# samuel-watson/glmmrMCML

Hardware: AMD Instinct MI355X
Metric: MCML iters/sec x m chains (simlik evals/sec) (higher is better)
Workload: dtype f64

## Files before the change

glmmrmcml_amd/csrc/ctx.h:

```cpp
#pragma once
#include "common.h"
#include "chol.h"
#include "covspec.h"
#include "band_plan.h"
#include "component_plan.h"
#include "step_ahead.h"

namespace mcml {

typedef int (*reduce_fn)(void* user, double* dev_buf, int n);

enum { KERNEL_SKINNY = 0, KERNEL_BAND = 1, KERNEL_DLDS = 2, KERNEL_REG = 3, KERNEL_SPARSE = 4, KERNEL_COMPONENT = 5,
       KERNEL_EXACT = 6,
       KERNEL_EXACT_COMPONENT = 7 };

struct StepRing {
    static constexpr int SLOTS = StepAhead::SLOTS;
    unsigned long long* h = nullptr;
    unsigned long long* d = nullptr;
    unsigned seq = 0;
    StepRing() = default;
    StepRing(const StepRing&) = delete;
    StepRing& operator=(const StepRing&) = delete;
    ~StepRing() { if (h) (void)hipHostFree(h); }
};

struct HmcState {
    StepRing ring;
    int C = 0;
    int Cw = 0;
    DevMat V, R, UP, GRAD, GRADP;
    DevMat MU, S;
    DevBuf chain;
    DevBuf partial;
    int partial_slots = 0;
    bool cm = false;
    DevBuf cm_part, cm_acc;
    DevBuf cm_part_fwd;
    DevMat LX, ZS;
    DevBuf cp_part;
};

constexpr int NUTS_MAXD = 12;
struct NutsState {
    DevMat vecs[16 + 4 * (NUTS_MAXD + 1)];
    DevBuf chain, part;
};

struct SparseZL {
    bool possible = false, active = false, built = false;
    int W = 0;
    long nnz = 0;
    DevBuf ell_col, ell_src, ell_z, ell_val;
    DevBuf csr_ptr, csr_i, csr_pos, csr_val;
    DevBuf row_start;
    bool factored = false;
    long nnz_z = 0, nnz_l = 0;
    DevBuf zcsr_ptr, zcsr_i, zcsr_val;
    DevBuf row_end;
    DevBuf blk_ptr;
    int nblk = 0, max_blk = 0;
};

struct ComponentDev {
    ComponentPlan plan;
    bool ready = false;
    DevBuf item_ptr, var_ptr, vars, slot_ptr, slot_quarter, slot_i, slot_src, slot_d;
};

struct CompFactors {
    DevBuf fac, fac_ptr, logdet;
    long long doubles = 0;
};

struct KernelProf {
    bool on = false;
    bool skip = false;
    long long seen[4] = {0, 0, 0, 0};
    std::vector<hipEvent_t> ev;
    std::vector<int> kind, e0, e1;
    size_t used = 0, nev = 0;
    int last_stop = -1;
    double ms[4] = {0, 0, 0, 0};
    long long cnt[4] = {0, 0, 0, 0};
    int fresh() {
        if (nev >= ev.size())
            for (int i = 0; i < 512; ++i) { hipEvent_t e; if (hipEventCreate(&e) != hipSuccess) return -1; ev.push_back(e); }
        return (int)nev++;
    }
    int begin(hipStream_t s, int k, bool chain = false) {
        if (!on) return -1;
        ++seen[k];
        if (skip) return -1;
        int st = (chain && last_stop >= 0) ? last_stop : fresh();
        if (st < 0) return -1;
        if (!(chain && last_stop >= 0)) (void)hipEventRecord(ev[st], s);
        if (used >= kind.size()) { kind.resize(used + 512); e0.resize(used + 512); e1.resize(used + 512); }
        kind[used] = k; e0[used] = st; e1[used] = -1;
        return (int)used++;
    }
    void end(hipStream_t s, int slot) {
        if (slot < 0) return;
        const int sp = fresh();
        if (sp < 0) return;
        (void)hipEventRecord(ev[sp], s);
        e1[slot] = sp; last_stop = sp;
    }
    void unchain() { last_stop = -1; }
    void collect() {
        for (size_t i = 0; i < used; ++i) {
            float t = 0;
            if (e1[i] >= 0 && hipEventElapsedTime(&t, ev[e0[i]], ev[e1[i]]) == hipSuccess) { ms[kind[i]] += t; cnt[kind[i]] += 1; }
        }
        used = 0; nev = 0; last_stop = -1;
    }
    ~KernelProf() { for (auto e : ev) (void)hipEventDestroy(e); }
// ... 168 lines not shown
```

glmmrmcml_amd/csrc/hmc.hip:

```cpp
#include <algorithm>
#include <atomic>
#include <chrono>
#include "entry.h"
#include "dgemm_mfma.h"
#include "dgemm_dlds.h"
#include "dgemm_band.h"
#include "dgemm_skinny.h"
#include "glm.h"
#include "reduce.h"
#include "rng.h"
#include "hmc_chain.h"
#include "hmc_cm.h"
#include "hmc_traj.h"

namespace mcml {

template <int FL>
struct EpiForwardT {
    double* MU; double* S; int ld; const double* xb; const double* y; int flink; int store_mu; double var_par;
    __device__ __forceinline__ double score(double yv, double mu) const {
        if constexpr (FL == 12) return glm_score_beta(yv, mu, var_par);
        else return glm_score(yv, mu, FL ? FL : flink);
    }
    __device__ __forceinline__ void elem(int m, int n, double accv) const {
// ... 77 lines not shown
                cb[r] = (size_t)nn * ld;
            }
            double xv[TM][4], rv[TM][4];
#pragma unroll
            for (int i = 0; i < TM; ++i) {
                const int m = mB + 16 * i + (lane & 15);
                const int mm = m < M ? m : 0;
#pragma unroll
                for (int r = 0; r < 4; ++r) {
                    xv[i][r] = Xs[mm + cb[r]];
                    rv[i][r] = mode == 1 ? R[mm + cb[r]] : 0.0;
                }
            }
#pragma unroll
            for (int r = 0; r < 4; ++r) {
                const double en = env[r];
                const bool more = s + 1 < stv[r];
#pragma unroll
                for (int i = 0; i < TM; ++i) {
                    const double x = xv[i][r];
                    double g = -1.0 * x;
                    g = g + post * acc[i][j][r];
                    acc[i][j][r] = g;
                    double rr = rv[i][r];
                    rr = rr + (en / 2) * g;
                    const double rr2 = rr + (en / 2) * g;
                    rr = more ? rr2 : rr;
                    rv[i][r] = rr;
                    xv[i][r] = x + en * rr;
                }
            }
#pragma unroll
            for (int r = 0; r < 4; ++r) {
                const bool act = inN[r] && (mode != 1 || s < stv[r]);
                if (!act) continue;
                const bool more = s + 1 < stv[r];
#pragma unroll
                for (int i = 0; i < TM; ++i) {
                    const int m = mB + 16 * i + (lane & 15);
                    if (m >= M) continue;
                    const size_t off = m + cb[r];
                    if (mode != 1 || !more) G[off] = acc[i][j][r];
                    if (mode == 1) {
                        if (more) UP[off] = xv[i][r];
                        R[off] = rv[i][r];
                    }
                }
            }
        }
    }
};

template <> struct BandFeed<EpiBackward> { static constexpr bool ok = true; };
template <> struct BandFeed<EpiForwardT<1>> { static constexpr bool ok = true; };
template <> struct BandFeed<EpiForwardT<3>> { static constexpr bool ok = true; };
template <> struct BandFeed<EpiForwardT<7>> { static constexpr bool ok = true; };


__global__ __launch_bounds__(256) void k_blockdiag_LV(int Q, int ncols, const int* start, const double* L, int ldl,
                                                      const double* V, int ldv, double* U, int ldu)
{
    const int q = blockIdx.x * 256 + threadIdx.x;
    if (q >= Q) return;
    const int s0 = start[q];
    for (int c = blockIdx.y; c < ncols; c += gridDim.y) {
        const double* v = V + (size_t)c * ldv;
        double acc = 0.0;
        for (int t = s0; t <= q; ++t) acc += L[q + (size_t)t * ldl] * v[t];
        U[q + (size_t)c * ldu] = acc;
    }
}

__global__ __launch_bounds__(256) void k_hmc_init(double* V, int ld, int Q, ChainArrays ca, uint64_t seed,
                                                  uint32_t chain_offset, uint32_t iter_idx, const double* inj_init)
{
    const int c = blockIdx.x;
    const uint32_t gid = chain_offset + (uint32_t)c;
    for (int q = threadIdx.x; q < Q; q += 256)
        V[q + (size_t)c * ld] = inj_init ? inj_init[q + (size_t)c * Q]
                                         : rng_normal(seed, (uint32_t)q, gid, 0u, 16u * iter_idx + 0u);
    if (threadIdx.x == 0) chain_reset(ca, c, seed, gid, iter_idx);
}

template <int FL>
__device__ __forceinline__ double chain_log_prob(const double* MU, int ldm, int n, const double* X, int ldx,
                                                 int Q, const double* y, double var_par, int flink_rt, int c,
                                                 double* sh)
{
    const int flink = FL ? FL : flink_rt;
    double ll = 0, lp = 0;
    for (int i0 = threadIdx.x; i0 < n; i0 += 1024) {
        double m4[4], y4[4];
#pragma unroll
        for (int u = 0; u < 4; ++u) {
            const int i = i0 + 256 * u;
            m4[u] = i < n ? MU[i + (size_t)c * ldm] : 0.0;
            y4[u] = i < n ? y[i] : 0.0;
        }
#pragma unroll
        for (int u = 0; u < 4; ++u)
            if (i0 + 256 * u < n) ll += glm_logpdf(y4[u], m4[u], var_par, flink);
    }
    for (int k0 = threadIdx.x; k0 < Q; k0 += 1024) {
        double x4[4];
#pragma unroll
        for (int u = 0; u < 4; ++u) { const int k = k0 + 256 * u; x4[u] = k < Q ? X[k + (size_t)c * ldx] : 0.0; }
#pragma unroll
        for (int u = 0; u < 4; ++u)
            if (k0 + 256 * u < Q) lp += glm_logpdf(x4[u], 0, 1, 7);
    }
    double a = block_sum(ll, sh);
    double b = block_sum(lp, sh);
    return a + b;
}

template <int FL>
__global__ __launch_bounds__(256) void k_hmc_lp0(const double* MU, int ldm, int n, const double* V, int ld, int Q,
                                                 const double* y, double var_par, int flink, double* lpcur)
{
    __shared__ double sh[4];
    double v = chain_log_prob<FL>(MU, ldm, n, V, ld, Q, y, var_par, flink, blockIdx.x, sh);
    if (threadIdx.x == 0) lpcur[blockIdx.x] = v;
}

__global__ __launch_bounds__(256) void k_hmc_propose(const double* V, const double* GRAD, double* R, double* UP,
                                                     int ld, int Q, ChainArrays ca, double lambda, int max_steps,
                                                     uint64_t seed, uint32_t chain_offset, uint32_t iter_idx,
                                                     int it, const double* inj_mom, int C)
{
    __shared__ double sh[4];
    const int c = blockIdx.x;
    const uint32_t gid = chain_offset + (uint32_t)c;
    const double e = ca.e[c];
    double ss = 0;
    for (int q = threadIdx.x; q < Q; q += 256) {
        const size_t off = q + (size_t)c * ld;
        double r = inj_mom ? inj_mom[q + ((size_t)it * C + c) * Q]
                           : rng_normal(seed, (uint32_t)q, gid, (uint32_t)it, 16u * iter_idx + 2u);
        ss += r * r;
        const double g = GRAD[off], v = V[off];
        r = r + (e / 2) * g;
        R[off] = r;
        UP[off] = v + e * r;
    }
    double tot = block_sum(ss, sh);
    if (threadIdx.x == 0) chain_begin_proposal(ca, c, tot, lambda, max_steps);
}

__global__ void k_max_steps(const int* steps, int C, int* out, unsigned long long* slot = nullptr, unsigned seq = 0)
{
    __shared__ int sh[256];
    int v = 0;
    for (int i = threadIdx.x; i < C; i += 256) v = max(v, steps[i]);
    sh[threadIdx.x] = v;
    __syncthreads();
    for (int o = 128; o > 0; o >>= 1) { if ((int)threadIdx.x < o) sh[threadIdx.x] = max(sh[threadIdx.x], sh[threadIdx.x + o]); __syncthreads(); }
    if (threadIdx.x == 0) {
        out[0] = sh[0];
        if (slot) __hip_atomic_store(slot, ((unsigned long long)seq << 32) | (unsigned)sh[0], __ATOMIC_RELEASE, __HIP_MEMORY_SCOPE_SYSTEM);
    }
}

template <int FL>
__global__ __launch_bounds__(256) void k_hmc_accept(double* V, double* GRAD, const double* R, const double* UP,
                                                    const double* GRADP, int ld, int Q, const double* MU, int ldm,
                                                    int n, const double* y, double var_par, int flink,
                                                    ChainArrays ca, double target_accept, int adapt, int it,
                                                    int C, uint8_t* flags, double* probs)
{
    __shared__ double sh[4];
    __shared__ int acc_s;
    const int c = blockIdx.x;
    double l2 = chain_log_prob<FL>(MU, ldm, n, UP, ld, Q, y, var_par, flink, c, sh);
    double kin = 0;
    for (int k0 = threadIdx.x; k0 < Q; k0 += 1024) {
        double r4[4];
#pragma unroll
        for (int u = 0; u < 4; ++u) { const int k = k0 + 256 * u; r4[u] = k < Q ? R[k + (size_t)c * ld] : 0.0; }
#pragma unroll
        for (int u = 0; u < 4; ++u)
            if (k0 + 256 * u < Q) kin += r4[u] * r4[u];
    }
    kin = block_sum(kin, sh);
    if (threadIdx.x == 0) acc_s = chain_decide(ca, c, l2, kin, target_accept, adapt, it, C, flags, probs);
    __syncthreads();
    const int acc = acc_s;
    if (acc)
        for (int k0 = threadIdx.x; k0 < Q; k0 += 1024) {
            double u4[4], g4[4];
#pragma unroll
            for (int u = 0; u < 4; ++u) {
                const int k = k0 + 256 * u;
                const size_t off = (k < Q ? k : 0) + (size_t)c * ld;
                u4[u] = UP[off]; g4[u] = GRADP[off];
            }
#pragma unroll
            for (int u = 0; u < 4; ++u) {
                const int k = k0 + 256 * u;
                if (k < Q) { const size_t off = k + (size_t)c * ld; V[off] = u4[u]; GRAD[off] = g4[u]; }
            }
        }
}

__global__ __launch_bounds__(256) void k_hmc_store(const double* V, int ld, int Q, double* SAMP, int lds,
                                                   int stride, int col)
{
    const int c = blockIdx.x;
    for (int k = threadIdx.x; k < Q; k += 256) SAMP[k + (size_t)(c * stride + col) * lds] = V[k + (size_t)c * ld];
}

__global__ void k_hmc_diag(ChainArrays ca, int C, double* out)
{
    if (threadIdx.x != 0 || blockIdx.x != 0) return;
    double sa = 0, se = 0, mn = 1e300, mx = 0, ms = 0, sl = 0;
    for (int c = 0; c < C; ++c) {
        sa += ca.acc[c]; se += ca.e[c];
        mn = fmin(mn, ca.e[c]); mx = fmax(mx, ca.e[c]);
        ms = fmax(ms, (double)ca.steps[c]); sl += (double)ca.leap[c];
    }
    out[0] = sa; out[1] = se; out[2] = mn; out[3] = mx; out[4] = ms; out[5] = sl;
}

static bool cm_traj_used(const Ctx& c) { return c.traj_mode == 1 && c.sp.active && c.cp.ready && c.cp.plan.feasible; }

static std::atomic<long long> g_traj_launches{0};
long long cm_traj_launch_count() { return g_traj_launches.load(); }

static int cm_traj_launch(Ctx& c, const TrajArgs& a)
{
    const CompView m = comp_view(c);
    const int waves = cp_waves(c.cp.plan, cp_forced_waves(CP_TRAJ_WAVES_ENV));
    const int lds = cp_lds_bytes(m.max_vars, waves);
    const dim3 grid(m.nitems, cm_chain_blocks(a.C));
    MCML_TRY((dispatch_flink<1, 3, 7, 12>(c.flink, [&](auto FL) {
        if (waves == 4) {
            MCML_TRY(ensure_dynamic_lds((const void*)k_cm_traj<FL(), 4>, cp_lds_bytes(CP_MAX_VARS, 4)));
            hipLaunchKernelGGL((k_cm_traj<FL(), 4>), grid, dim3(256), lds, c.stream, m, a);
        } else {
            MCML_TRY(ensure_dynamic_lds((const void*)k_cm_traj<FL(), 1>, cp_lds_bytes(CP_MAX_VARS, 1)));
            hipLaunchKernelGGL((k_cm_traj<FL(), 1>), grid, dim3(64), lds, c.stream, m, a);
        }
        return (int)MCML_OK;
    })));
    MCML_HIP(hipGetLastError());
    ++g_traj_launches;
    return MCML_OK;
}

static int hmc_alloc(Ctx& c, int C)
{
    HmcState& h = c.hmc;
    h.C = C; h.Cw = C;
    h.cm = c.sp.active;
    auto mat = [&](DevMat& m, int len) { return h.cm ? m.alloc(C, len) : m.alloc(len, C); };
    for (DevMat* m : {&h.V, &h.R, &h.UP, &h.GRAD, &h.GRADP}) MCML_TRY(mat(*m, c.Q));
    MCML_TRY(mat(h.MU, c.n)); MCML_TRY(mat(h.S, c.n));
    MCML_TRY(h.chain.ensure(sizeof(double) * (size_t)round_up(C, 16) * 8));
    if (h.cm) {
        const size_t nchn = (size_t)(c.n + CM_ROWS - 1) / CM_ROWS, nchq = (size_t)(c.Q + cm_qrows(c.Q) - 1) / cm_qrows(c.Q);
        MCML_TRY(h.cm_part.ensure(sizeof(double) * (nchn + 3 * nchq + 4) * (size_t)h.V.ld));
        MCML_TRY(h.cm_acc.ensure(sizeof(int) * (size_t)round_up(C, 64)));
        if (c.sp.factored) { MCML_TRY(h.LX.alloc(C, c.Q)); MCML_TRY(h.ZS.alloc(C, c.Q)); }
        if (cm_traj_used(c)) MCML_TRY(h.cp_part.ensure(sizeof(double) * 4 * (size_t)c.cp.plan.nitems() * h.V.ld));
        return MCML_OK;
    }
    MCML_HIP(hipMemsetAsync(h.V.d(), 0, sizeof(double) * (size_t)h.V.ld * C, c.stream));
    MCML_HIP(hipMemsetAsync(h.UP.d(), 0, sizeof(double) * (size_t)h.UP.ld * C, c.stream));
    MCML_HIP(hipMemsetAsync(h.S.d(), 0, sizeof(double) * (size_t)h.S.ld * C, c.stream));
    return MCML_OK;
}

static bool use_dlds()
{
    static int v = -1;
    if (v < 0) { const char* e = getenv("GLMMR_MCML_GEMM"); v = (e && !strcmp(e, "reg")) ? 0 : 1; }
    return v == 1;
}

static bool use_skinny()
{
    const char* e = getenv("GLMMR_MCML_SKINNY");
    return !(e && !strcmp(e, "0"));
}

struct DenseOp { BandPlan& plan; bool band; int M, K; const DevMat& A; };
template <class Epi>
static int dense_product(Ctx& c, int dir, const DenseOp& a, const double* B, int ldb, const Epi& epi)
{
    const int N = c.hmc.Cw, lda = a.A.ld;
    const double* A = a.A.d();
    if (use_skinny() && skinny_applicable(a.plan, a.M, a.K, N, lda)) {
        c.last_kernel[dir] = KERNEL_SKINNY;
        return launch_skinny(c.stream, a.plan, N, A, lda, B, ldb, epi);
    }
    if (a.band && dlds_applicable(a.M, N, a.K, A, lda, a.A.cols_alloc, B, ldb)) {
        c.last_kernel[dir] = KERNEL_BAND;
        return launch_gemm_band(c.stream, a.plan, N, A, lda, B, ldb, epi);
    }
    if (use_dlds() && dlds_applicable(a.M, N, a.K, A, lda, a.A.cols_alloc, B, ldb)) {
        c.last_kernel[dir] = KERNEL_DLDS;
        return launch_gemm_dlds(c.stream, a.M, N, a.K, A, lda, B, ldb, epi);
    }
    c.last_kernel[dir] = KERNEL_REG;
    return launch_gemm<false>(c.stream, a.M, N, a.K, A, lda, B, ldb, epi);
}

enum : unsigned {
    PROD_STORE_MU = 1,
    PROD_CHAIN = 2,
    PROD_WANT_LL = 4,
    PROD_LX_READY = 8,
};

static int hmc_forward(Ctx& c, const double* X, int ldx, double var_par, unsigned flags = PROD_STORE_MU)
{
    HmcState& h = c.hmc;
    const int store_mu = (flags & PROD_STORE_MU) ? 1 : 0;
    const int slot = c.prof.begin(c.stream, 0, (flags & PROD_CHAIN) != 0);
    int rc;
    if (h.cm) {
        c.last_kernel[0] = KERNEL_SPARSE;
        const int rpw = CM_FR;
        dim3 grid((c.n + 4 * rpw - 1) / (4 * rpw), (h.Cw + 63) / 64);
        int W = c.sp.W; const int* col = c.sp.ell_col.as<int>(); const double* val = c.sp.ell_val.d(); const double* Xin = X;
        if (c.sp.factored) {
            if (!(flags & PROD_LX_READY))
            hipLaunchKernelGGL(k_cm_Lrow, dim3((c.Q + 3) / 4, (h.Cw + 63) / 64), dim3(256), 0, c.stream, c.Q, h.Cw, h.V.ld,
                               c.sp.row_start.as<int>(), c.L.d(), c.L.ld, X, h.LX.d());
            W = c.z_width; col = c.z_idx.as<int>(); val = c.z_val.d(); Xin = h.LX.d();
        }
        double* pll = nullptr;
        if (flags & PROD_WANT_LL) {
            MCML_TRY(h.cm_part_fwd.ensure(sizeof(double) * (size_t)grid.x * h.V.ld));
            pll = h.cm_part_fwd.d();
        }
        dispatch_flink<1, 3, 7, 12>(c.flink, [&](auto FL) {
            hipLaunchKernelGGL((k_cm_forward<FL()>), grid, dim3(256), 0, c.stream, c.n, h.Cw, h.V.ld, W, col, val, Xin, c.xb.d(),
                               c.y.d(), c.flink, var_par, store_mu, h.MU.d(), h.S.d(), rpw, pll, h.V.ld);
        });
        rc = (hipGetLastError() == hipSuccess) ? MCML_OK : MCML_EHIP;
    } else
        rc = dispatch_flink<1, 3, 7, 12>(c.flink, [&](auto FL) {
            return dense_product(c, 0, DenseOp{c.plan_fwd, c.band_fwd, c.n, c.Q, c.ZL}, X, ldx,
                                 EpiForwardT<FL()>{h.MU.d(), h.S.d(), h.MU.ld, c.xb.d(), c.y.d(), c.flink, store_mu, var_par});
        });
    c.prof.end(c.stream, slot);
    return rc;
}

static int hmc_backward(Ctx& c, const double* Xs, double* G, int s, double var_par, int mode, unsigned flags = 0,
                        int next_lx = 0)
{
    HmcState& h = c.hmc;
    ChainArrays ca = chain_arrays(h);
    EpiBackward epi{Xs, G, h.R.d(), h.UP.d(), h.V.ld, ca.e, ca.steps, s, glm_score_post(var_par, c.flink), mode};
    const int slot = c.prof.begin(c.stream, 1, (flags & PROD_CHAIN) != 0);
    int rc;
    if (h.cm) {
        const bool f = c.sp.factored;
        const int* ptr = f ? c.sp.zcsr_ptr.as<int>() : c.sp.csr_ptr.as<int>();
        const int* ci = f ? c.sp.zcsr_i.as<int>() : c.sp.csr_i.as<int>();
        const double* cv = f ? c.sp.zcsr_val.d() : c.sp.csr_val.d();
        double* out = f ? h.ZS.d() : G;
        const int m1 = f ? 2 : mode;
// ... 104 lines not shown
    const int Q = c.Q;
    MCML_TRY(c.U.alloc(Q, ncols));
    MCML_HIP(hipMemsetAsync(c.U.d(), 0, sizeof(double) * (size_t)c.U.ld * ncols, c.stream));
    if (c.sp.active && c.sp.row_start.p) {
        int gy = ncols < 1024 ? ncols : 1024;
        hipLaunchKernelGGL(k_blockdiag_LV, dim3((Q + 255) / 256, gy), dim3(256), 0, c.stream, Q, ncols,
                           c.sp.row_start.as<int>(), c.L.d(), c.L.ld, samp.d(), samp.ld, c.U.d(), c.U.ld);
        MCML_HIP(hipGetLastError());
    } else {
        EpiAxpby epi{c.U.d(), c.U.ld, 1.0, 0.0};
        MCML_TRY(launch_gemm<false>(c.stream, Q, ncols, Q, c.L.d(), c.L.ld, samp.d(), samp.ld, epi));
    }
    c.mcols = ncols;
    c.zu_valid = false; c.uall_valid = false;
    return MCML_OK;
}

}

#include "hmc_exact.h"
#include "hmc_exact_comp.h"

namespace mcml {

bool hmc_exact_applicable(const Ctx& c) { return exact_applicable(c); }
int hmc_exact_sample(Ctx& c, const double* beta, double var_par, const glmmr_mcml_hmc_opts* o, uint64_t seed, uint32_t iter_idx,
                     const double* inj_z, glmmr_mcml_hmc_diag* diag, int* ncols_out)
{
    return exact_gaussian_sample(c, beta, var_par, o, seed, iter_idx, inj_z, nullptr, nullptr, diag, ncols_out);
}

bool hmc_exact_component_applicable(const Ctx& c) { return exact_component_applicable(c); }
int hmc_exact_component_sample(Ctx& c, const double* beta, double var_par, const glmmr_mcml_hmc_opts* o, uint64_t seed,
                               uint32_t iter_idx, const double* inj_z, glmmr_mcml_hmc_diag* diag, int* ncols_out)
{
    return exact_component_sample(c, beta, var_par, o, seed, iter_idx, inj_z, nullptr, nullptr, diag, ncols_out);
}
void hmc_exact_component_sizes(const Ctx& c, long long* out3)
{
    const ComponentPlan& p = c.cp.plan;
    const int waves = cp_waves(p, cp_forced_waves(CP_LA_WAVES_ENV));
    out3[0] = waves; out3[1] = exc_lds_bytes(p.max_vars); out3[2] = 8LL * comp_factor_doubles(c);
}

struct HmcTiming {
    using Clock = std::chrono::steady_clock;
    enum { PROPOSE, LOOK_AHEAD, TRAJECTORY, ACCEPT, NSEG };
    const bool on = enabled();
    Clock::time_point t_phase = Clock::now(), t_mark = t_phase, t_prop = t_phase;
    double setup = 0, loop = 0, sync = 0, slowest = 0, seg[NSEG] = {};
    int n_sync = 0, nprop = 0;

    static bool enabled() { static const bool v = getenv("GLMMR_MCML_HMC_TIMING") != nullptr; return v; }
    static double since(Clock::time_point t) { return std::chrono::duration<double, std::milli>(Clock::now() - t).count(); }
    static double now_ms() { return std::chrono::duration<double, std::milli>(Clock::now().time_since_epoch()).count(); }
    double phase_end() { const double d = since(t_phase); t_phase = Clock::now(); return d; }
    void proposal()
    {
        if (!on) return;
        if (nprop++ > 0) slowest = std::max(slowest, since(t_prop));
        t_prop = t_mark = Clock::now();
    }
    void start() { if (on) t_mark = Clock::now(); }
    void mark(int k) { if (on) { seg[k] = std::max(seg[k], since(t_mark)); t_mark = Clock::now(); } }
    void waited() { if (on) { sync += since(t_mark); ++n_sync; } }
    void print(int total) const
    {
        if (on)
            fprintf(stderr, "hmc_sample: set-up %.2f ms | %d proposals %.2f ms enqueue (%d synchronous, %.2f ms waiting; slowest proposal %.2f ms: propose %.2f, count look-ahead %.2f, trajectory %.2f, accept %.2f) | tail %.2f ms\n",
                    setup, total, loop, n_sync, sync, slowest, seg[PROPOSE], seg[LOOK_AHEAD], seg[TRAJECTORY], seg[ACCEPT], since(t_phase));
    }
};

struct HmcCall {
    const glmmr_mcml_hmc_opts* o; double var_par; uint64_t seed; uint32_t iter_idx;
    SampleShape sh;
    ChainArrays ca;
    const double* mom; uint8_t* flags; double* probs;
    const DevMat* samp;
    int lf;
    double* tpart; size_t tstride;
    StepRing* ring; int* d_maxs;
    bool pending_commit;
    int adapt(int it) const { return (it < o->warmup) && (it < o->adapt); }
};

static void commit_cm(Ctx& c, HmcCall& k, int it)
{
    HmcState& h = c.hmc;
    int stride;
    const bool stores_now = k.sh.column_of(it, &stride) >= 0;
    if (it + 1 < k.sh.total && !stores_now) k.pending_commit = true;
    else hipLaunchKernelGGL(k_cm_commit, dim3((k.sh.C + 63) / 64, cm_parts(c).nchq), dim3(256), 0, c.stream, h.V.d(), h.GRAD.d(),
                            h.UP.d(), h.GRADP.d(), h.V.ld, c.Q, k.sh.C, h.cm_acc.as<int>());
}

static void store_draw(Ctx& c, const HmcCall& k, int it)
{
    int stride;
    const int col = k.sh.column_of(it, &stride);
    if (col >= 0) store_columns(c, *k.samp, stride, col);
}

static int leapfrog_steps(Ctx& c, const HmcCall& k, StepAhead& ahead, HmcTiming& t, int it)
{
    HmcState& h = c.hmc;
    StepRing& ring = *k.ring;
    const unsigned seq = ++ring.seq;
    const int slot = (int)(seq % StepRing::SLOTS);
    hipLaunchKernelGGL(k_max_steps, dim3(1), dim3(256), 0, c.stream, k.ca.steps, k.sh.C, k.d_maxs, ring.d + slot, seq);
    MCML_HIP(hipGetLastError());
    t.mark(HmcTiming::PROPOSE);
    int maxs = ahead.launched(seq, HmcTiming::now_ms);
    if (maxs != StepAhead::SYNCHRONISE) t.mark(HmcTiming::LOOK_AHEAD);
    else {
        t.start();
        MCML_HIP(hipStreamSynchronize(c.stream));
        t.waited();
        maxs = ahead.synchronised(seq);
        MCML_REQUIRE(maxs != StepAhead::NOT_ARRIVED, "hmc: the step count of proposal %d did not arrive (token %llx, expected sequence %u)", it, ring.h[slot], seq);
        MCML_REQUIRE(maxs != StepAhead::OUT_OF_ORDER, "hmc: step-count ring out of order");
    }
    MCML_REQUIRE(maxs >= 1 && maxs <= k.o->max_steps, "hmc: step count %d out of range", maxs);
    c.prof.skip = (it & 3) != 0;
    t.start();
    int rc = MCML_OK;
    for (int s = 0; s < maxs && rc == MCML_OK; ++s) {
        const bool last = s == maxs - 1;
        rc = hmc_forward(c, h.UP.d(), h.UP.ld, k.var_par, (s > 0 ? PROD_CHAIN : 0) | (last ? (h.cm ? PROD_WANT_LL : PROD_STORE_MU) : 0) |
                                                              (k.lf && s > 0 ? PROD_LX_READY : 0));
        if (rc == MCML_OK) rc = hmc_backward(c, h.UP.d(), h.GRADP.d(), s, k.var_par, 1, PROD_CHAIN, last ? 0 : k.lf);
    }
    c.prof.skip = false;
    t.mark(HmcTiming::TRAJECTORY);
    MCML_TRY(rc);
    c.prof.unchain();
    return MCML_OK;
}

static int propose_dense(Ctx& c, HmcCall& k, StepAhead& ahead, HmcTiming& t, int it)
{
    HmcState& h = c.hmc;
    const glmmr_mcml_hmc_opts* o = k.o;
    hipLaunchKernelGGL(k_hmc_propose, dim3(k.sh.C), dim3(256), 0, c.stream, h.V.d(), h.GRAD.d(), h.R.d(), h.UP.d(),
                       h.V.ld, c.Q, k.ca, o->lambda, o->max_steps, k.seed, (uint32_t)o->chain_offset, k.iter_idx, it,
                       k.mom, k.sh.C);
    MCML_TRY(leapfrog_steps(c, k, ahead, t, it));
    dispatch_flink<1, 3, 7>(c.flink, [&](auto FL) {
        hipLaunchKernelGGL((k_hmc_accept<FL()>), dim3(k.sh.C), dim3(256), 0, c.stream, h.V.d(), h.GRAD.d(), h.R.d(), h.UP.d(),
                           h.GRADP.d(), h.V.ld, c.Q, h.MU.d(), h.MU.ld, c.n, c.y.d(), k.var_par, c.flink, k.ca,
                           o->target_accept, k.adapt(it), it, k.sh.C, k.flags, k.probs);
    });
    store_draw(c, k, it);
    MCML_HIP(hipGetLastError());
    t.mark(HmcTiming::ACCEPT);
    return MCML_OK;
}

static int propose_cm(Ctx& c, HmcCall& k, StepAhead& ahead, HmcTiming& t, int it)
{
    HmcState& h = c.hmc;
    const glmmr_mcml_hmc_opts* o = k.o;
    const CmParts p = cm_parts(c);
    const dim3 chains((k.sh.C + 63) / 64);
    hipLaunchKernelGGL(k_cm_propose, dim3(chains.x, p.nchq), dim3(256), 0, c.stream, h.V.d(), h.GRAD.d(), h.R.d(),
                       h.UP.d(), h.V.ld, c.Q, k.sh.C, k.ca, k.seed, (uint32_t)o->chain_offset, k.iter_idx, it, k.mom,
                       p.ss, p.ldp, k.pending_commit ? h.cm_acc.as<int>() : nullptr, h.GRADP.d());
    k.pending_commit = false;
    hipLaunchKernelGGL(k_cm_propose_fin, chains, dim3(256), 0, c.stream, p.ss, p.nchq, p.ldp, k.sh.C, k.ca, o->lambda, o->max_steps);
    MCML_TRY(leapfrog_steps(c, k, ahead, t, it));
    MCML_TRY(cm_logprob_partials(c, h.UP.d(), h.R.d(), k.var_par, true));
    hipLaunchKernelGGL((k_cm_accept_fin<false>), chains, dim3(256), 0, c.stream, h.cm_part_fwd.d(), p.lp, p.kin,
                       cm_fwd_chunks(c), p.nchq, p.ldp, k.sh.C, k.ca, o->target_accept, k.adapt(it), it, k.flags, k.probs,
                       h.cm_acc.as<int>(), (const double*)nullptr, 0, 0.0, 0);
    commit_cm(c, k, it);
    store_draw(c, k, it);
    MCML_HIP(hipGetLastError());
    t.mark(HmcTiming::ACCEPT);
    return MCML_OK;
}

static int propose_component(Ctx& c, HmcCall& k, int it)
{
    HmcState& h = c.hmc;
    const glmmr_mcml_hmc_opts* o = k.o;
    double* const tpart = k.tpart; const size_t tstride = k.tstride;
    TrajArgs a{h.V.d(), h.GRAD.d(), h.UP.d(), h.GRADP.d(), h.V.ld, k.sh.C, c.Q, k.ca, k.seed, (uint32_t)o->chain_offset,
               k.iter_idx, it, k.mom, k.pending_commit ? h.cm_acc.as<int>() : nullptr, o->lambda, o->max_steps, c.flink,
               k.var_par, glm_score_post(k.var_par, c.flink), tpart, tpart + tstride, tpart + 2 * tstride,
               tpart + 3 * tstride, h.V.ld};
    k.pending_commit = false;
    c.prof.skip = (it & 3) != 0;
    const int slot = c.prof.begin(c.stream, 0);
    const int rc = cm_traj_launch(c, a);
    c.prof.end(c.stream, slot);
    c.prof.skip = false;
    c.prof.unchain();
    MCML_TRY(rc);
    const int ni = c.cp.plan.nitems();
    hipLaunchKernelGGL((k_cm_accept_fin<true>), dim3((k.sh.C + 63) / 64), dim3(256), 0, c.stream, tpart + tstride, tpart + 2 * tstride,
                       tpart + 3 * tstride, ni, ni, h.V.ld, k.sh.C, k.ca, o->target_accept, k.adapt(it), it, k.flags, k.probs,
                       h.cm_acc.as<int>(), tpart, ni, o->lambda, o->max_steps);
    commit_cm(c, k, it);
    store_draw(c, k, it);
    MCML_HIP(hipGetLastError());
    c.last_kernel[0] = c.last_kernel[1] = KERNEL_COMPONENT;
    return MCML_OK;
}

int hmc_sample(Ctx& c, const double* beta, double var_par, const glmmr_mcml_hmc_opts* o, uint64_t seed,
               uint32_t iter_idx, const double* inj_init, const double* inj_mom, uint8_t* flags_out,
               double* probs_out, glmmr_mcml_hmc_diag* diag, int* ncols_out)
{
    MCML_REQUIRE(c.n > 0 && c.have_L && (c.ZL.d() || c.sp.active), "hmc: model / L not set (call update_L or set_L first)");
    MCML_REQUIRE(o && o->warmup >= 0 && o->nsamp > 0 && o->max_steps >= 1 && o->lambda > 0,
                 "hmc: bad options");
    MCML_REQUIRE(beta, "hmc: beta is null");
    if ((c.draws_mode == 1 || c.draws_mode == 2) && exact_applicable(c))
        return exact_gaussian_sample(c, beta, var_par, o, seed, iter_idx, nullptr, flags_out, probs_out, diag, ncols_out);
    if (c.draws_mode == 2 && exact_component_applicable(c))
        return exact_component_sample(c, beta, var_par, o, seed, iter_idx, nullptr, flags_out, probs_out, diag, ncols_out);
    const SampleShape sh = sample_shape(o->nsamp, o->warmup, o->chains);
    const int C = sh.C, total = sh.total, ncols = sh.ncols;
    const int Q = c.Q;
    HmcState& h = c.hmc;
    HmcTiming t;
    MCML_TRY(model_update_beta(c, beta));
    MCML_TRY(hmc_alloc(c, C));
    DevMat samp;
    MCML_TRY(samp.alloc(Q, ncols));
    MCML_HIP(hipMemsetAsync(samp.d(), 0, sizeof(double) * (size_t)samp.ld * ncols, c.stream));

    DevBuf d_init, d_mom, d_flags, d_probs;
    if (inj_init) {
        MCML_TRY(d_init.ensure(sizeof(double) * (size_t)Q * C));
        MCML_TRY(copy_h2d(d_init.p, inj_init, sizeof(double) * (size_t)Q * C, c.stream));
    }
    if (inj_mom) {
        MCML_TRY(d_mom.ensure(sizeof(double) * (size_t)Q * C * total));
        MCML_TRY(copy_h2d(d_mom.p, inj_mom, sizeof(double) * (size_t)Q * C * total, c.stream));
    }
    if (flags_out) MCML_TRY(d_flags.ensure((size_t)C * total));
    if (probs_out) MCML_TRY(d_probs.ensure(sizeof(double) * (size_t)C * total));

    static const bool spec_allowed = !(getenv("GLMMR_MCML_HMC_SPEC") && atoi(getenv("GLMMR_MCML_HMC_SPEC")) == 0);
    StepRing& ring = h.ring;
    if (!ring.h) {
        MCML_HIP(hipHostMalloc((void**)&ring.h, sizeof(unsigned long long) * StepRing::SLOTS, hipHostMallocMapped | hipHostMallocCoherent));
        memset(ring.h, 0, sizeof(unsigned long long) * StepRing::SLOTS);
        MCML_HIP(hipHostGetDevicePointer((void**)&ring.d, ring.h, 0));
    }
    StepAhead ahead(ring.h, ring.seq, o->max_steps, spec_allowed);

    const bool traj = h.cm && cm_traj_used(c);
    HmcCall k{o, var_par, seed, iter_idx, sh, chain_arrays(h), d_mom.d(), d_flags.as<uint8_t>(), d_probs.d(), &samp,
              h.cm ? cm_fuse_width(c) : 0, traj ? h.cp_part.d() : nullptr, traj ? (size_t)c.cp.plan.nitems() * h.V.ld : 0,
              &ring, c.scalars.as<int>() + 34, false};

    MCML_TRY(sampler_init_state(c, seed, (uint32_t)o->chain_offset, iter_idx, d_init.d()));
    MCML_TRY(hmc_eval_state(c, var_par));
    if (sh.single_chain_layout && o->warmup == 0) store_columns(c, samp, 0, 0);
    if (traj) MCML_TRY(comp_fill_xy(c));
    t.setup = t.phase_end();
    for (int it = 0; it < total; ++it) {
        t.proposal();
        if (traj) MCML_TRY(propose_component(c, k, it));
        else if (h.cm) MCML_TRY(propose_cm(c, k, ahead, t, it));
        else MCML_TRY(propose_dense(c, k, ahead, t, it));
    }
    t.loop = t.phase_end();
    MCML_TRY(samples_to_U(c, samp, ncols));
    c.niter = sh.niter;
    if (flags_out) MCML_TRY(copy_d2h(flags_out, d_flags.p, (size_t)C * total, c.stream));
    if (probs_out) MCML_TRY(copy_d2h(probs_out, d_probs.p, sizeof(double) * (size_t)C * total, c.stream));
    double dg[6] = {0, 0, 0, 0, 0, 0};
    hipLaunchKernelGGL(k_hmc_diag, dim3(1), dim3(64), 0, c.stream, k.ca, C, c.scalars.d() + 8);
    MCML_TRY(copy_d2h(dg, c.scalars.d() + 8, sizeof dg, c.stream));
    MCML_HIP(hipStreamSynchronize(c.stream));
    t.print(total);
    c.prof.collect();
    if (diag) {
        diag->accept_rate = dg[0] / ((double)C * total);
        diag->mean_e = dg[1] / C; diag->min_e = dg[2]; diag->max_e = dg[3];
        diag->max_steps_used = (int)dg[4]; diag->leapfrog_total = (long long)dg[5];
    }
    if (ncols_out) *ncols_out = ncols;
    return MCML_OK;
}

int hmc_dbg_log_prob_grad(Ctx& c, const double* beta, double var_par, const double* V, int ncols, double* lp,
                          double* G)
{
    MCML_REQUIRE(c.n > 0 && c.have_L && (c.ZL.d() || c.sp.active), "log_prob_grad: model / L not set");
    MCML_TRY(model_update_beta(c, beta));
    MCML_TRY(hmc_alloc(c, ncols));
    HmcState& h = c.hmc;
    ChainArrays ca = chain_arrays(h);
    if (h.cm) {
        DevMat tmp;
        MCML_TRY(tmp.alloc(c.Q, ncols));
        MCML_TRY(copy_h2d_2d(tmp.d(), sizeof(double) * tmp.ld, V, sizeof(double) * c.Q, sizeof(double) * c.Q, ncols, c.stream));
        hipLaunchKernelGGL(k_cm_transpose, dim3((ncols + 31) / 32, (c.Q + 31) / 32), dim3(256), 0, c.stream, tmp.d(), tmp.ld,
                           ncols, c.Q, h.V.d(), (size_t)h.V.ld, (size_t)1, 0);
        MCML_HIP(hipGetLastError());
        MCML_TRY(hmc_eval_state(c, var_par));
        hipLaunchKernelGGL(k_cm_transpose, dim3((c.Q + 31) / 32, (ncols + 31) / 32), dim3(256), 0, c.stream, h.GRAD.d(), h.GRAD.ld,
                           c.Q, ncols, tmp.d(), (size_t)tmp.ld, (size_t)1, 0);
        MCML_HIP(hipGetLastError());
        MCML_TRY(copy_d2h(lp, ca.lpcur, sizeof(double) * ncols, c.stream));
        MCML_TRY(download_matrix(G, c.Q, tmp.d(), tmp.ld, c.Q, ncols, c.stream));
        return c.sync();
    }
    MCML_TRY(copy_h2d_2d(h.V.d(), sizeof(double) * h.V.ld, V, sizeof(double) * c.Q, sizeof(double) * c.Q, ncols, c.stream));
    MCML_TRY(hmc_eval_state(c, var_par));
    MCML_TRY(copy_d2h(lp, ca.lpcur, sizeof(double) * ncols, c.stream));
    return download_matrix(G, c.Q, h.GRAD.d(), h.GRAD.ld, c.Q, ncols, c.stream);
}

}

#include "nuts.h"
```

glmmrmcml_amd/csrc/hmc_chain.h:

```cpp
#pragma once
#include "../../include/glmmr_mcml_c.h"
#include "ctx.h"
#include "rng.h"

namespace mcml {

struct ChainArrays {
    double *e, *ebar, *H, *lpcur, *K0;
    int *steps, *acc;
    uint32_t* gen;
    long long* leap;
};

inline ChainArrays chain_arrays(const HmcState& h)
{
    ChainArrays a;
    const size_t C = (size_t)round_up(h.C, 16);
    double* d = h.chain.d();
    a.e = d; a.ebar = d + C; a.H = d + 2 * C; a.lpcur = d + 3 * C; a.K0 = d + 4 * C;
    a.leap = reinterpret_cast<long long*>(d + 5 * C);
    a.steps = reinterpret_cast<int*>(d + 6 * C);
    a.acc = a.steps + C;
    a.gen = reinterpret_cast<uint32_t*>(a.acc + C);
    return a;
}

__device__ __forceinline__ void chain_reset(const ChainArrays& ca, int c, uint64_t seed, uint32_t gid, uint32_t iter_idx)
{
    ca.e[c] = 0.001; ca.ebar[c] = 1.0; ca.H[c] = 0.0; ca.acc[c] = 0; ca.leap[c] = 0;
    ca.gen[c] = chain_minstd_seed(seed, gid, iter_idx);
    ca.steps[c] = 1;
}

__device__ __forceinline__ int chain_step_count(double lambda, double e, int max_steps)
{
    double st = round(lambda / e);
    if (!(st >= 1.0)) st = 1.0;
    if (st > (double)max_steps) st = (double)max_steps;
    return (int)st;
}

__device__ __forceinline__ void chain_begin_proposal(const ChainArrays& ca, int c, double sum_r2, double lambda, int max_steps)
{
    ca.K0[c] = 0.5 * sum_r2;
    const int st = chain_step_count(lambda, ca.e[c], max_steps);
    ca.steps[c] = st;
    ca.leap[c] += (long long)st;
}

__device__ __forceinline__ int chain_decide(const ChainArrays& ca, int c, double l2, double kin, double target_accept, int adapt,
                                            int it, int C, uint8_t* flags, double* probs)
{
    const double lprt = 0.5 * kin, lpr = ca.K0[c], l1 = ca.lpcur[c];
    const double prob = fmin(1.0, exp(-l1 + lpr + l2 - lprt));
    uint32_t g = ca.gen[c];
    const double runif = minstd_canonical(g);
    ca.gen[c] = g;
    const int acc = runif < prob;
    if (acc) { ca.lpcur[c] = l2; ca.acc[c] += 1; }
    if (flags) flags[c + (size_t)it * C] = (uint8_t)acc;
    if (probs) probs[c + (size_t)it * C] = prob;
    if (adapt) {
        const int iter = it + 1;
        const double f1 = 1.0 / (iter + 10);
        const double H = (1 - f1) * ca.H[c] + f1 * (target_accept - prob);
        ca.H[c] = H;
        const double loge = -4.60517 - (sqrt((double)iter / 0.05)) * H;
        const double powm = pow((double)iter, -0.75);
        const double logbare = powm * loge + (1 - powm) * log(ca.ebar[c]);
        ca.e[c] = exp(loge);
        ca.ebar[c] = exp(logbare);
    } else {
        ca.e[c] = ca.ebar[c];
    }
    return acc;
}

struct SampleShape {
    int C, d, total, ncols, niter, warmup;
    bool single_chain_layout;
    int column_of(int it, int* stride) const
    {
        *stride = single_chain_layout ? 0 : d;
        if (single_chain_layout) return it >= warmup - 1 ? it - warmup + 1 : -1;
        return it >= warmup ? it - warmup : -1;
    }
};
inline SampleShape sample_shape(int nsamp, int warmup, int chains, bool nuts = false)
{
    SampleShape s;
    s.C = chains > 0 ? chains : 1;
    s.single_chain_layout = s.C == 1 && !nuts;
    s.d = (nsamp + s.C - 1) / s.C;
    s.warmup = warmup; s.total = warmup + s.d;
    s.ncols = s.single_chain_layout ? s.d + 1 : s.C * s.d;
    s.niter = s.single_chain_layout ? s.d : s.ncols;
    return s;
}
__host__ __device__ __forceinline__ void draw_of_column(int j, int C, int d, uint32_t* chain, uint32_t* draw)
{
    *chain = C > 1 ? (uint32_t)(j / d) : 0u;
    *draw = C > 1 ? (uint32_t)(j % d) : (uint32_t)j;
}

inline void exact_finish(const SampleShape& s, uint8_t* flags_out, double* probs_out, glmmr_mcml_hmc_diag* diag, int* ncols_out)
{
    const size_t np = (size_t)s.C * s.total;
    if (flags_out) memset(flags_out, 1, np);
// ... 11 lines not shown
```

Baseline: 1231.

## Fuse HMC accept, next-proposal momentum draw and max-steps reduction into one turn kernel

Adds a per-chain 'turn' kernel that performs the accept/reject decision for iteration it and then immediately begins the next proposal: it draws fresh momentum, does the half-step and position update, and computes the step count. A last-block atomic ticket replaces the separate k_max_steps launch and publishes the max step count to the host ring. Momentum draws are optionally stashed in shared memory and generated while the log-prob loop runs, to hide RNG latency. This removes two kernel launches and one pass over V/GRAD per iteration. In exchange it adds device atomics, shared-memory pressure and buffer swaps that must stay consistent with the leapfrog path.

```diff
diff --git a/glmmrmcml_amd/csrc/ctx.h b/glmmrmcml_amd/csrc/ctx.h
--- a/glmmrmcml_amd/csrc/ctx.h
+++ b/glmmrmcml_amd/csrc/ctx.h
@@ -32,6 +32,7 @@
     DevMat V, R, UP, GRAD, GRADP;
     DevMat MU, S;
     DevBuf chain;
+    DevBuf turn_call;
     DevBuf partial;
     int partial_slots = 0;
     bool cm = false;
diff --git a/glmmrmcml_amd/csrc/hmc.hip b/glmmrmcml_amd/csrc/hmc.hip
--- a/glmmrmcml_amd/csrc/hmc.hip
+++ b/glmmrmcml_amd/csrc/hmc.hip
@@ -183,10 +183,11 @@
     if (threadIdx.x == 0) chain_reset(ca, c, seed, gid, iter_idx);
 }
 
-template <int FL>
+struct NothingUnder { __device__ __forceinline__ void operator()(int) const {} };
+template <int FL, class Under = NothingUnder>
 __device__ __forceinline__ double chain_log_prob(const double* MU, int ldm, int n, const double* X, int ldx,
                                                  int Q, const double* y, double var_par, int flink_rt, int c,
-                                                 double* sh)
+                                                 double* sh, Under under = Under())
 {
     const int flink = FL ? FL : flink_rt;
     double ll = 0, lp = 0;
@@ -206,6 +207,7 @@
         double x4[4];
 #pragma unroll
         for (int u = 0; u < 4; ++u) { const int k = k0 + 256 * u; x4[u] = k < Q ? X[k + (size_t)c * ldx] : 0.0; }
+        under(k0);
 #pragma unroll
         for (int u = 0; u < 4; ++u)
             if (k0 + 256 * u < Q) lp += glm_logpdf(x4[u], 0, 1, 7);
@@ -303,6 +305,130 @@
         }
 }
 
+constexpr size_t TURN_STASH_BYTES = 40000;
+struct TurnCall {
+    double* chain; int Cpad;
+    int C; double target_accept; uint8_t* flags; double* probs;
+    double lambda; int max_steps;
+    int* out; unsigned long long* ring;
+};
+__global__ void k_hmc_turn_call(const TurnCall v, TurnCall* dst) { if (threadIdx.x == 0) *dst = v; }
+
+struct TurnArgs {
+    double *V, *GRAD, *R, *UP, *GRADP; int ld, Q;
+    const double* MU; int ldm, n; const double* y; double var_par; int flink;
+    uint64_t seed; uint32_t chain_offset, iter_idx; const double* inj_mom; int C;
+    int it, adapt; unsigned seq;
+    const TurnCall* call;
+};
+
+template <int FL, bool STASH>
+__device__ __forceinline__ void hmc_turn(const TurnArgs& a, double* draws)
+{
+    __shared__ double sh[4];
+    __shared__ double e_s;
+    __shared__ int acc_s;
+    const int c = blockIdx.x, Q = a.Q, ld = a.ld;
+    const uint32_t gid = a.chain_offset + (uint32_t)c;
+    const size_t col = (size_t)c * ld;
+    auto draw = [&](int k) {
+        return rng_normal(a.seed, (uint32_t)k, gid, (uint32_t)(a.it + 1), 16u * a.iter_idx + 2u);
+    };
+    double kin = 0;
+    const double l2 = chain_log_prob<FL>(a.MU, a.ldm, a.n, a.UP, ld, Q, a.y, a.var_par, a.flink, c, sh, [&](int k0) {
+        double r4[4];
+#pragma unroll
+        for (int u = 0; u < 4; ++u) { const int k = k0 + 256 * u; r4[u] = k < Q ? a.R[k + col] : 0.0; }
+        if constexpr (STASH) {
+#pragma nounroll
+            for (int k = k0; k < k0 + 1024 && k < Q; k += 256) draws[k] = draw(k);
+        }
+#pragma unroll
+        for (int u = 0; u < 4; ++u)
+            if (k0 + 256 * u < Q) kin += r4[u] * r4[u];
+    });
+    kin = block_sum(kin, sh);
+    if (threadIdx.x == 0) {
+        const TurnCall& k = *a.call;
+        const ChainArrays ca = chain_arrays(k.chain, (size_t)k.Cpad);
+        acc_s = chain_decide(ca, c, l2, kin, k.target_accept, a.adapt, a.it, k.C, k.flags, k.probs);
+        e_s = ca.e[c];
+    }
+    __syncthreads();
+    const int acc = acc_s;
+    const double e = e_s;
+    const double* sv = acc ? a.UP : a.V;
+    const double* sg = acc ? a.GRADP : a.GRAD;
+    double ss = 0;
+    for (int k0 = threadIdx.x; k0 < Q; k0 += 1024) {
+        double v4[4], g4[4], r4[4];
+#pragma unroll
+        for (int u = 0; u < 4; ++u) {
+            const int k = k0 + 256 * u;
+            r4[u] = 0.0;
+            if constexpr (STASH) { if (k < Q) r4[u] = draws[k]; }
+            else if (k < Q && a.inj_mom) r4[u] = a.inj_mom[k + ((size_t)(a.it + 1) * a.C + c) * Q];
+        }
+        if constexpr (!STASH)
+            if (!a.inj_mom) {
+#pragma nounroll
+                for (int u = 0; u < 4; ++u) {
+                    const int k = k0 + 256 * u;
+                    const double r = k < Q ? draw(k) : 0.0;
+#pragma unroll
+                    for (int w = 0; w < 4; ++w) r4[w] = w == u ? r : r4[w];
+                }
+            }
+#pragma unroll
+        for (int u = 0; u < 4; ++u) {
+            const int k = k0 + 256 * u;
+            const size_t off = (k < Q ? k : 0) + col;
+            v4[u] = sv[off]; g4[u] = sg[off];
+        }
+#pragma unroll
+        for (int u = 0; u < 4; ++u) {
+            const int k = k0 + 256 * u;
+            if (k >= Q) continue;
+            const size_t off = k + col;
+            double r = r4[u];
+            ss += r * r;
+            r = r + (e / 2) * g4[u];
+            a.R[off] = r;
+            a.V[off] = v4[u] + e * r;
+            if (!acc) { a.UP[off] = v4[u]; a.GRADP[off] = g4[u]; }
+        }
+    }
+    const double tot = block_sum(ss, sh);
+    if (threadIdx.x == 0) {
+        const TurnCall& k = *a.call;
+        const ChainArrays ca = chain_arrays(k.chain, (size_t)k.Cpad);
+        chain_begin_proposal(ca, c, tot, k.lambda, k.max_steps);
+        int* const count = k.out + 2;
+        __hip_atomic_fetch_max(count, ca.steps[c], __ATOMIC_RELAXED, __HIP_MEMORY_SCOPE_AGENT);
+        const int ticket = __hip_atomic_fetch_add(count + 1, 1, __ATOMIC_ACQ_REL, __HIP_MEMORY_SCOPE_AGENT);
+        if (ticket == k.C - 1) {
+            const int m = __hip_atomic_load(count, __ATOMIC_RELAXED, __HIP_MEMORY_SCOPE_AGENT);
+            k.out[0] = m;
+            __hip_atomic_store(count, 0, __ATOMIC_RELAXED, __HIP_MEMORY_SCOPE_AGENT);
+            __hip_atomic_store(count + 1, 0, __ATOMIC_RELAXED, __HIP_MEMORY_SCOPE_AGENT);
+            __hip_atomic_store(k.ring + a.seq % StepRing::SLOTS, ((unsigned long long)a.seq << 32) | (unsigned)m, __ATOMIC_RELEASE,
+                               __HIP_MEMORY_SCOPE_SYSTEM);
+        }
+    }
+}
+template <int FL>
+__global__ __launch_bounds__(256) __attribute__((amdgpu_waves_per_eu(4))) void k_hmc_turn(const TurnArgs a)
+{
+    extern __shared__ double draws[];
+    static_assert(FL != 0, "no stash with the run-time family / link code: glm_logpdf's switch needs 302 registers (see chain_log_prob)");
+    hmc_turn<FL, true>(a, draws);
+}
+template <int FL>
+__global__ __launch_bounds__(256) void k_hmc_turn_plain(const TurnArgs a)
+{
+    hmc_turn<FL, false>(a, nullptr);
+}
+
 __global__ __launch_bounds__(256) void k_hmc_store(const double* V, int ld, int Q, double* SAMP, int lds,
                                                    int stride, int col)
 {
@@ -381,6 +507,12 @@
 static bool use_skinny()
 {
     const char* e = getenv("GLMMR_MCML_SKINNY");
+    return !(e && !strcmp(e, "0"));
+}
+
+static bool turn_enabled()
+{
+    const char* e = getenv("GLMMR_MCML_HMC_TURN");
     return !(e && !strcmp(e, "0"));
 }
 
@@ -651,6 +783,8 @@
     double* tpart; size_t tstride;
     StepRing* ring; int* d_maxs;
     bool pending_commit;
+    bool turn;
+    bool turned;
     int adapt(int it) const { return (it < o->warmup) && (it < o->adapt); }
 };
 
@@ -677,8 +811,10 @@
     StepRing& ring = *k.ring;
     const unsigned seq = ++ring.seq;
     const int slot = (int)(seq % StepRing::SLOTS);
-    hipLaunchKernelGGL(k_max_steps, dim3(1), dim3(256), 0, c.stream, k.ca.steps, k.sh.C, k.d_maxs, ring.d + slot, seq);
-    MCML_HIP(hipGetLastError());
+    if (!k.turned) {
+        hipLaunchKernelGGL(k_max_steps, dim3(1), dim3(256), 0, c.stream, k.ca.steps, k.sh.C, k.d_maxs, ring.d + slot, seq);
+        MCML_HIP(hipGetLastError());
+    }
     t.mark(HmcTiming::PROPOSE);
     int maxs = ahead.launched(seq, HmcTiming::now_ms);
     if (maxs != StepAhead::SYNCHRONISE) t.mark(HmcTiming::LOOK_AHEAD);
@@ -707,19 +843,43 @@
     return MCML_OK;
 }
 
+static void turn_dense(Ctx& c, HmcCall& k, int it)
+{
+    HmcState& h = c.hmc;
+    const glmmr_mcml_hmc_opts* o = k.o;
+    const unsigned seq = k.ring->seq + 1;
+    const bool stash = !k.mom && sizeof(double) * (size_t)c.Q <= TURN_STASH_BYTES;
+    const dim3 grid(k.sh.C), block(256);
+    const TurnArgs a{h.V.d(), h.GRAD.d(), h.R.d(), h.UP.d(), h.GRADP.d(), h.V.ld, c.Q, h.MU.d(), h.MU.ld, c.n, c.y.d(),
+                     k.var_par, c.flink, k.seed, (uint32_t)o->chain_offset, k.iter_idx, k.mom, k.sh.C, it, k.adapt(it), seq,
+                     h.turn_call.as<TurnCall>()};
+    dispatch_flink<1, 3, 7>(c.flink, [&](auto FL) {
+        if constexpr (FL() != 0)
+            if (stash) { hipLaunchKernelGGL(k_hmc_turn<FL()>, grid, block, sizeof(double) * (size_t)c.Q, c.stream, a); return; }
+        hipLaunchKernelGGL(k_hmc_turn_plain<FL()>, grid, block, 0, c.stream, a);
+    });
+    std::swap(h.V, h.UP);
+    std::swap(h.GRAD, h.GRADP);
+    k.turned = true;
+}
+
 static int propose_dense(Ctx& c, HmcCall& k, StepAhead& ahead, HmcTiming& t, int it)
 {
     HmcState& h = c.hmc;
     const glmmr_mcml_hmc_opts* o = k.o;
-    hipLaunchKernelGGL(k_hmc_propose, dim3(k.sh.C), dim3(256), 0, c.stream, h.V.d(), h.GRAD.d(), h.R.d(), h.UP.d(),
-                       h.V.ld, c.Q, k.ca, o->lambda, o->max_steps, k.seed, (uint32_t)o->chain_offset, k.iter_idx, it,
-                       k.mom, k.sh.C);
+    if (!k.turned)
+        hipLaunchKernelGGL(k_hmc_propose, dim3(k.sh.C), dim3(256), 0, c.stream, h.V.d(), h.GRAD.d(), h.R.d(), h.UP.d(),
+                           h.V.ld, c.Q, k.ca, o->lambda, o->max_steps, k.seed, (uint32_t)o->chain_offset, k.iter_idx, it,
+                           k.mom, k.sh.C);
     MCML_TRY(leapfrog_steps(c, k, ahead, t, it));
-    dispatch_flink<1, 3, 7>(c.flink, [&](auto FL) {
-        hipLaunchKernelGGL((k_hmc_accept<FL()>), dim3(k.sh.C), dim3(256), 0, c.stream, h.V.d(), h.GRAD.d(), h.R.d(), h.UP.d(),
-                           h.GRADP.d(), h.V.ld, c.Q, h.MU.d(), h.MU.ld, c.n, c.y.d(), k.var_par, c.flink, k.ca,
-                           o->target_accept, k.adapt(it), it, k.sh.C, k.flags, k.probs);
-    });
+    k.turned = false;
+    if (k.turn && it + 1 < k.sh.total) turn_dense(c, k, it);
+    else
+        dispatch_flink<1, 3, 7>(c.flink, [&](auto FL) {
+            hipLaunchKernelGGL((k_hmc_accept<FL()>), dim3(k.sh.C), dim3(256), 0, c.stream, h.V.d(), h.GRAD.d(), h.R.d(), h.UP.d(),
+                               h.GRADP.d(), h.V.ld, c.Q, h.MU.d(), h.MU.ld, c.n, c.y.d(), k.var_par, c.flink, k.ca,
+                               o->target_accept, k.adapt(it), it, k.sh.C, k.flags, k.probs);
+        });
     store_draw(c, k, it);
     MCML_HIP(hipGetLastError());
     t.mark(HmcTiming::ACCEPT);
@@ -824,7 +984,14 @@
     const bool traj = h.cm && cm_traj_used(c);
     HmcCall k{o, var_par, seed, iter_idx, sh, chain_arrays(h), d_mom.d(), d_flags.as<uint8_t>(), d_probs.d(), &samp,
               h.cm ? cm_fuse_width(c) : 0, traj ? h.cp_part.d() : nullptr, traj ? (size_t)c.cp.plan.nitems() * h.V.ld : 0,
-              &ring, c.scalars.as<int>() + 34, false};
+              &ring, c.scalars.as<int>() + 34, false, !h.cm && turn_enabled(), false};
+    if (k.turn) {
+        MCML_HIP(hipMemsetAsync(k.d_maxs + 2, 0, 2 * sizeof(int), c.stream));
+        MCML_TRY(h.turn_call.ensure(sizeof(TurnCall)));
+        const TurnCall tc{h.chain.d(), round_up(C, 16), C, o->target_accept, k.flags, k.probs, o->lambda, o->max_steps, k.d_maxs, ring.d};
+        hipLaunchKernelGGL(k_hmc_turn_call, dim3(1), dim3(64), 0, c.stream, tc, h.turn_call.as<TurnCall>());
+        MCML_HIP(hipGetLastError());
+    }
 
     MCML_TRY(sampler_init_state(c, seed, (uint32_t)o->chain_offset, iter_idx, d_init.d()));
     MCML_TRY(hmc_eval_state(c, var_par));
diff --git a/glmmrmcml_amd/csrc/hmc_chain.h b/glmmrmcml_amd/csrc/hmc_chain.h
--- a/glmmrmcml_amd/csrc/hmc_chain.h
+++ b/glmmrmcml_amd/csrc/hmc_chain.h
@@ -12,11 +12,9 @@
     long long* leap;
 };
 
-inline ChainArrays chain_arrays(const HmcState& h)
+__host__ __device__ inline ChainArrays chain_arrays(double* d, size_t C)
 {
     ChainArrays a;
-    const size_t C = (size_t)round_up(h.C, 16);
-    double* d = h.chain.d();
     a.e = d; a.ebar = d + C; a.H = d + 2 * C; a.lpcur = d + 3 * C; a.K0 = d + 4 * C;
     a.leap = reinterpret_cast<long long*>(d + 5 * C);
     a.steps = reinterpret_cast<int*>(d + 6 * C);
@@ -24,6 +22,7 @@
     a.gen = reinterpret_cast<uint32_t*>(a.acc + C);
     return a;
 }
+inline ChainArrays chain_arrays(const HmcState& h) { return chain_arrays(h.chain.d(), (size_t)round_up(h.C, 16)); }
 
 __device__ __forceinline__ void chain_reset(const ChainArrays& ca, int c, uint64_t seed, uint32_t gid, uint32_t iter_idx)
 {
```

Result: no change. 1233 (median of 4 runs) (+0.2%).
